# bitmagier/q-learning

Measured on AMD Instinct MI355X. Metric: env-steps/sec + grad-updates/sec, Breakout 84×84×4, 1/2/4/8 MI355X, higher is better.
Workload: dtype fp32; 1 GPU; C3: 8192 Breakout envs per GPU, replay 1000000 per GPU in HBM (prefilled), Nature-DQN (3 conv + 2 dense) in fp32, B=1024, update every 128 env-steps per GPU (replay ratio 8 samples/env-step), epsilon-greedy acting; envs_per_gpu=8192, batch=1024, replay_capacity=1000000, update_after_actions=128, parallelism=single, rccl_world=1, global_batch_per_update=1024, env_dtype=fp32 physics, u8 frames, qnet_dtype=fp32 (exact-fp32 MFMA v_mfma_f32_16x16x4_f32)

## Files before the change

### q-learning_amd/csrc/qnet32.hip

```cpp
#include <hip/hip_ext.h>
#include <hip/hip_runtime.h>

#include <algorithm>
#include <cmath>
#include <cstdlib>
#include <map>
#include <tuple>
#include <vector>

#include "objects.h"
#include "profiler.h"
#include "qnet.h"
#include "qnet32_kernels.h"
#include "update32_dev.h"

namespace qlx {

using namespace q32;

struct F32Net {
  bool bg_rows = true;
  int c1_skip = 1;
  bool update_scheduled = false;
  bool dense_partials = false;
  float partials_scale = 1.0f;
  float *fa1 = nullptr, *fa2 = nullptr, *fa3 = nullptr, *fa4 = nullptr;
  float* fpart = nullptr;
  int *frl2 = nullptr, *frl3 = nullptr;
  unsigned long long* frcnt = nullptr;
  float* fbgc = nullptr;
  uint32_t* fsteps = nullptr;
  uint8_t* fneed = nullptr;
  int fneed_ld = 0;
  uint32_t* frows2 = nullptr;
  uint8_t* fbg2 = nullptr;
  uint32_t* frows3 = nullptr;
  uint8_t* fbg3 = nullptr;
  int fparity = 0;
  int frl_cap = 0;
  int fchunk = 0;
  DeviceBuffer<uint8_t> fgrad;
  int fgrad_batch = 0;
  float *fdz1 = nullptr, *fdz2 = nullptr, *fdz3 = nullptr, *fdz4 = nullptr;
  float *fslab1 = nullptr, *fslab2 = nullptr, *fslab3 = nullptr;
  float* fpb1 = nullptr;
  float* fpbg2 = nullptr;
  float* fs2 = nullptr;
  float* fpbg3 = nullptr;
  float* fs3 = nullptr;
};

constexpr int kHeadPitch = 514;
template <int MODE, int HS = 16>
__global__ __launch_bounds__(256) void k_head32(Fc2Args A) {
  __shared__ f32x4 part[4][16];
  __shared__ float gsh[16];
  __shared__ int ash[16];
  __shared__ __attribute__((aligned(16))) float xs[16 * kHeadPitch];
  __shared__ __attribute__((aligned(16))) float w4s[512 * 3];
  typedef float f32x2 __attribute__((ext_vector_type(2)));
  const int lane = threadIdx.x & 63, wave = threadIdx.x >> 6;
  const int s0 = blockIdx.x * HS;
  const int j = lane & 15, g = lane >> 4, n = lane & 15;
  const int b = s0 + j;
  const bool valid = j < HS && b < A.B;
  const bool tail = wave == 0 && g == 0 && valid;
  const int bt = tail ? b : 0;
  int t_act = 0;
  float t_y = 0.0f, t_w = 1.0f, t_r = 0.0f, t_qs[3] = {0.0f, 0.0f, 0.0f};
  bool t_done = false;
  if (tail) {
    if (MODE == 3) {
      t_act = A.actions[bt];
      t_y = A.y[bt];
      if (A.weights) t_w = A.weights[bt];
    } else if (MODE == 2) {
      t_r = A.rewards[bt];
      t_done = A.dones[bt] != 0;
      if (A.q_select)
        for (int r = 0; r < 3; ++r) t_qs[r] = A.q_select[bt * 3 + r];
    }
// ... 418 lines not shown
  if ((int)blockIdx.x < nconv) conv_adam_block(A, N, blockIdx.x);
  else AdamDense{A, ndense}.run((int)blockIdx.x - nconv, nrm);
}

static int conv_adam_blocks() {
  int n = 0;
  for (int v = 0; v < 6; ++v) n += (kVarSize[v] + kConvAdamChunk - 1) / kConvAdamChunk;
  return n;
}



static int segs_of(int v) { return (kVarSize[v] + kNormSeg - 1) / kNormSeg; }
static_assert((1605632 + kNormSeg - 1) / kNormSeg <= kNormSegMax, "norm partials per variable");
static_assert((36864 + kNormSeg - 1) / kNormSeg <= 4 * kConvSegsPerGroup && (32768 + kNormSeg - 1) / kNormSeg <= 4 * kConvSegsPerGroup,
              "conv variable segments per conv_adam_block");
static_assert((512 * 3 + kNormSeg - 1) / kNormSeg <= 64 && (32768 + kNormSeg - 1) / kNormSeg <= 64 &&
              (36864 + kNormSeg - 1) / kNormSeg <= 64 && (8192 + kNormSeg - 1) / kNormSeg <= 64, "<= 64 partials but W3");

static int num_cus();

constexpr int kC1MaxIt = 64;
static int c1_blocks(int n) { return std::max(std::min(n, 2 * num_cus()), (n + kC1MaxIt - 1) / kC1MaxIt); }
static bool c1_one(int n) { return n <= 2048; }
static int c1_grid(int n) { return c1_one(n) ? n : c1_blocks(n); }

void f32_create(qlx_model* m) {
  F32Net& w = *(m->fp32 = new F32Net);
  const char* bg = std::getenv("QLX_F32_BG");
  w.bg_rows = !(bg && bg[0] == '0');
  const char* sk = std::getenv("QLX_F32_C1_SKIP");
  w.c1_skip = (sk && sk[0] == '0') ? 0 : 1;
}

void f32_destroy(qlx_model* m) {
  delete m->fp32;
  m->fp32 = nullptr;
}

void f32_workspace(qlx_model* m, int B) {
  F32Net& w = *m->fp32;
  const int C = std::min(B, kF32FwdChunk);
  static_assert((uint64_t)kF32FwdChunk * 12800 * 4 < 0x80000000ull, "a forward chunk's a1 stays below 2^31 bytes");
  int nseg = 0;
  for (int v = 0; v < kNumVars; ++v) nseg += segs_of(v);
  const int frl_cap = C + kListSlots * (C / std::max(1, std::min(C, 2 * num_cus())) + 1) +
                      std::max(2 * num_cus(), C / kC1MaxIt + 1) + kListSlots;
  const int need_ld = (C + 63) / 64 * 64;
  ws_alloc(m, B, [&](Arena& a) {
    w.fa1 = a.take<float>((size_t)C * 12800); w.fa2 = a.take<float>((size_t)C * 5184); w.fa3 = a.take<float>((size_t)C * 3136);
    w.fa4 = a.take<float>((size_t)B * 512);
    w.fpart = a.take<float>(nseg);
    w.frl2 = a.take<int>((size_t)frl_cap * 81); w.frl3 = a.take<int>((size_t)frl_cap * 49);
    w.frcnt = a.take<unsigned long long>(2 * 2 * kListSlots * kCntStride);
    w.fbgc = a.take<float>(160);
    w.fsteps = a.take<uint32_t>((size_t)C * 4);
    w.fneed = a.take<uint8_t>((size_t)100 * need_ld);
    w.frows2 = a.take<uint32_t>((size_t)C * 4); w.fbg2 = a.take<uint8_t>((size_t)81 * need_ld);
    w.frows3 = a.take<uint32_t>((size_t)C * 4); w.fbg3 = a.take<uint8_t>((size_t)49 * need_ld);
  });
  QLX_HIP(hipMemset(w.frcnt, 0, 2 * 2 * kListSlots * kCntStride * 8));
  w.fneed_ld = need_ld;
  w.frl_cap = frl_cap;
  w.fparity = 0;
  w.fchunk = C;
}

static void f32_grad_workspace(qlx_model* m, int B) {
  F32Net& w = *m->fp32;
  if (B <= w.fgrad_batch) return;
  QLX_HIP(hipStreamSynchronize(m->stream));
  w.fgrad.release();
  w.fgrad_batch = 0;
  auto layout = [&](Arena& a) {
    w.fdz1 = a.take<float>((size_t)B * 12800); w.fdz2 = a.take<float>((size_t)B * 5184); w.fdz3 = a.take<float>((size_t)B * 3136);
    w.fdz4 = a.take<float>((size_t)B * 512);
    w.fslab1 = a.take<float>((size_t)((B + kSC1 - 1) / kSC1) * 257 * 32);
    w.fslab2 = a.take<float>((size_t)((B + kSC2 - 1) / kSC2) * 513 * 64);
    w.fslab3 = a.take<float>((size_t)((B + kSC3 - 1) / kSC3) * 577 * 64);
    w.fpb1 = a.take<float>((size_t)((B + 15) / 16) * 400 * 32);
    w.fpbg2 = a.take<float>((size_t)((B + 15) / 16) * 81 * 64); w.fs2 = a.take<float>((size_t)((B + 15) / 16) * 64);
    w.fpbg3 = a.take<float>((size_t)((B + 15) / 16) * 49 * 64); w.fs3 = a.take<float>((size_t)((B + 15) / 16) * 64);
  };
  Arena size;
  layout(size);
  w.fgrad.alloc(size.off);
  Arena a{(uintptr_t)w.fgrad.get()};
  layout(a);
  w.fgrad_batch = B;
}

template <class P>
static void launch(qlx_model* m, const P& p, const char* scope, double work, hipStream_t s) {
  hipEvent_t ea = nullptr, eb = nullptr;
  if (m->prof) m->prof->ext(scope, work, &ea, &eb);
  hipExtLaunchKernelGGL(k_gemm32<P>, dim3(p.g.blocks()), dim3(threads_of<P>()), gemm_lds_bytes<P>(), s, ea, eb, 0u, p);
  QLX_HIP(hipGetLastError());
  debug_sync(s, scope);
}

template <class P1, class P2, class S, class T = NoSide>
static void launch_pair(qlx_model* m, const P1& p1, const P2& p2, const S& side, const char* scope, double work, hipStream_t s,
                        const T& tail = T{}) {
  const size_t lds = std::max({gemm_lds_bytes<P1>(), gemm_lds_bytes<P2>(), S::LDS, T::LDS});
  hipEvent_t ea = nullptr, eb = nullptr;
  if (m->prof) m->prof->ext(scope, work, &ea, &eb);
// ... 18 lines not shown
  return n;
}

static Grid grid(int M, int BM, int N, int BN, int nz) { return Grid{(M + BM - 1) / BM, (N + BN - 1) / BN, nz}; }

static int c1_skip(const qlx_model* m) { return m->fp32->c1_skip; }

static int balanced_whole_tiles(int M) {
  const int ncu = num_cus(), t = M / 64, whole = t - t % ncu;
  if (whole < ncu || M - whole * 64 > 32 * ncu) return 0;
  return whole;
}

template <class P, class S>
static void launch_list(qlx_model* m, const P& p, const S& side, const char* scope, double work, hipStream_t s) {
  hipEvent_t ea = nullptr, eb = nullptr;
  if (m->prof) m->prof->ext(scope, work, &ea, &eb);
  const size_t lds = std::max(gemm_lds_bytes<P>(), S::LDS);
  hipExtLaunchKernelGGL((k_gemm32_side<P, S>), dim3(side.blocks() + p.g.blocks()), dim3(threads_of<P>()), lds, s, ea, eb, 0u, p, side);
  QLX_HIP(hipGetLastError());
  debug_sync(s, scope);
}

static bool bg_rows(const qlx_model* m) { return m->fp32->bg_rows; }

static bool c1_sparse_dz(const qlx_model* m) { return bg_rows(m) && c1_skip(m); }
template <class PW, class PR, class PF>
static void conv_fwd(qlx_model* m, int M, const float* in, const float* wt, const float* bias, float* out, const char* scope,
                     double work, hipStream_t s, const PF& plain) {
  const int whole = balanced_whole_tiles(M);
  if (!whole) {
    launch(m, plain, scope, work, s);
    return;
  }
  const PW pw{Grid{whole, 1, 1}, in, wt, bias, out, M};
  const PR pr{{Grid{(M - whole * 64 + 15) / 16, 1, 1}, in, wt, bias, out, M}, whole * 4};
  launch_pair(m, pw, pr, NoSide{}, scope, work, s);
}

void f32_forward(qlx_model* m, const uint8_t* const* table, int B, hipStream_t s) {
  F32Net& w = *m->fp32;
  QLX_CHECK(m->ws_batch >= B, QLX_E_STATE, "f32 forward: workspace too small");
  m->last_batch = B;
  const float* p = m->d_params;
  for (int c0 = 0; c0 < B; c0 += w.fchunk) {
    const int n = std::min(w.fchunk, B - c0);
    const bool big = n > 2048;
    const bool lists = bg_rows(m);
    unsigned long long* cnt = w.frcnt + 2 * kListSlots * kCntStride * w.fparity;
    const bool one = c1_one(n);
    const int G = c1_grid(n);
    const int per_slot = ((G + kListSlots - 1) / kListSlots) * ((n + G - 1) / G);
    const int cap2 = per_slot * 81, cap3 = per_slot * 49;
    QLX_CHECK((size_t)kListSlots * cap2 <= w.frl_cap * 81, QLX_E_STATE, "row lists too small");
    const C1Lists L{lists ? w.frl2 : nullptr, w.frl3, cap2, cap3, cnt, w.frcnt + 2 * kListSlots * kCntStride * (w.fparity ^ 1),
                    w.fbgc, w.fsteps, w.fneed, w.fneed_ld, w.frows2, w.fbg2, w.frows3, w.fbg3};
    if (lists) w.fparity ^= 1;
    {
      const char* sc = big ? "f32_conv1_fwd_big" : "f32_conv1_fwd";
      hipEvent_t ea = nullptr, eb = nullptr;
      if (m->prof) m->prof->ext(sc, 2.0 * n * 400 * 32 * 256, &ea, &eb);
      auto kern = one ? k_conv1_fwd32<0, true> : k_conv1_fwd32<1>;
      QLX_CHECK((n + G - 1) / G <= (one ? 1 : kC1MaxIt), QLX_E_STATE, "conv1 forward: too many samples per block");
      const size_t frames = (one ? 1 : 2) * kC1Frames;
      const size_t lds = frames + 3 * kC1RmDw * 4 + (size_t)((n + G - 1) / G) * 6 * 8 + 8;
      set_lds_limit((const void*)kern, frames + 3 * kC1RmDw * 4 + (size_t)(one ? 1 : kC1MaxIt) * 6 * 8 + 8);
      hipExtLaunchKernelGGL(kern, dim3(G), dim3(256), lds, s, ea, eb, 0u, table + (size_t)c0 * 4, n,
                            p + var_offset(0), p + var_offset(1), w.fa1, c1_skip(m), L);
      QLX_HIP(hipGetLastError());
      debug_sync(s, sc);
    }
    if (lists) {
      const int nw = std::min(256, std::max(16, n / 16));
      float* c2 = w.fbgc + 32;
      float* c3 = w.fbgc + 96;
      const BgRows2 s23{{nw, w.frl2, cnt, cap2, c2, w.fa2}, {nw, w.frl3, cnt + kCntStride, cap3, c3, w.fa3}};
      auto lgrid = [&](int cap, int BM, int BN) { return Grid{1 + kListSlots * ((cap + BM - 1) / BM), 64 / BN, 1}; };
      auto run = [&](auto t2, auto t3, const char* sc2, const char* sc3) {
        using P2 = decltype(t2);
        using P3 = decltype(t3);
        const ConstRows cr{{w.fbgc, p + var_offset(2), p + var_offset(3), c2}, {c2, p + var_offset(4), p + var_offset(5), c3}};
        P2 p2{lgrid(cap2, P2::BM, P2::BN), w.fa1, p + var_offset(2), p + var_offset(3), w.fa2, w.frl2, cap2, cnt, w.fbgc};
        p2.pre_batched = big;
        launch_list(m, p2, cr, sc2, 2.0 * n * 81 * 64 * 512, s);
        launch_list(m, P3{lgrid(cap3, P3::BM, P3::BN), w.fa2, p + var_offset(4), p + var_offset(5), w.fa3, w.frl3, cap3, cnt + kCntStride, c2},
                    s23, sc3, 2.0 * n * 49 * 64 * 576, s);
      };
      if (big) {
        run(PConv2FwdL<64, 64, 2, 2>{}, PConv3FwdL<64, 64, 2, 2>{}, "f32_conv2_fwd_big", "f32_conv3_fwd_big");
        launch(m, PFc1FwdB{grid(n, PFc1FwdB::BM, 512, PFc1FwdB::BN, 1), w.fa3, p + var_offset(6), p + var_offset(7), w.fa4 + (size_t)c0 * 512, n}, "f32_fc1_fwd_big",
               2.0 * n * 3136 * 512, s);
      } else {
        run(PConv2FwdL<64, 64, 2, 2>{}, PConv3FwdL<32, 64, 2, 2>{}, "f32_conv2_fwd", "f32_conv3_fwd");
        launch(m, PFc1FwdS{grid(n, PFc1FwdS::BM, 512, PFc1FwdS::BN, 1), w.fa3, p + var_offset(6), p + var_offset(7), w.fa4 + (size_t)c0 * 512, n}, "f32_fc1_fwd",
               2.0 * n * 3136 * 512, s);
      }
    } else if (big) {
      launch(m, PConv2Fwd{grid(n * 81, 64, 64, 64, 1), w.fa1, p + var_offset(2), p + var_offset(3), w.fa2, n * 81}, "f32_conv2_fwd_big",
             2.0 * n * 81 * 64 * 512, s);
      launch(m, PConv3Fwd{grid(n * 49, 64, 64, 64, 1), w.fa2, p + var_offset(4), p + var_offset(5), w.fa3, n * 49}, "f32_conv3_fwd_big",
             2.0 * n * 49 * 64 * 576, s);
      launch(m, PFc1FwdB{grid(n, PFc1FwdB::BM, 512, PFc1FwdB::BN, 1), w.fa3, p + var_offset(6), p + var_offset(7), w.fa4 + (size_t)c0 * 512, n}, "f32_fc1_fwd_big",
             2.0 * n * 3136 * 512, s);
    } else {
      conv_fwd<PConv2Fwd, PConv2FwdR>(m, n * 81, w.fa1, p + var_offset(2), p + var_offset(3), w.fa2, "f32_conv2_fwd", 2.0 * n * 81 * 64 * 512, s,
                                      PConv2FwdS{grid(n * 81, 64, 64, 32, 1), w.fa1, p + var_offset(2), p + var_offset(3), w.fa2, n * 81});
      conv_fwd<PConv3Fwd, PConv3FwdR>(m, n * 49, w.fa2, p + var_offset(4), p + var_offset(5), w.fa3, "f32_conv3_fwd", 2.0 * n * 49 * 64 * 576, s,
                                      PConv3FwdS{grid(n * 49, 64, 64, 32, 1), w.fa2, p + var_offset(4), p + var_offset(5), w.fa3, n * 49});
      launch(m, PFc1FwdS{grid(n, PFc1FwdS::BM, 512, PFc1FwdS::BN, 1), w.fa3, p + var_offset(6), p + var_offset(7), w.fa4 + (size_t)c0 * 512, n}, "f32_fc1_fwd",
             2.0 * n * 3136 * 512, s);
    }
  }
}

void f32_head(int mode, const Fc2Args& a, int B, hipStream_t s) {
  constexpr int kHs3 = 4;
  const dim3 g((B + 15) / 16), blk(256);
  switch (mode) {
    case 0: hipLaunchKernelGGL(k_head32<0>, g, blk, 0, s, a); break;
    case 1: hipLaunchKernelGGL(k_head32<1>, g, blk, 0, s, a); break;
    case 2: hipLaunchKernelGGL(k_head32<2>, g, blk, 0, s, a); break;
    default: hipLaunchKernelGGL((k_head32<3, kHs3>), dim3((B + kHs3 - 1) / kHs3), blk, 0, s, a); break;
  }
  QLX_HIP(hipGetLastError());
  debug_sync(s, "k_head32");
}

Fc2Args f32_fc2_args(qlx_model* m, int B) {
  Fc2Args a = fc2_common(m, B);
  a.a4f = m->fp32->fa4;
  return a;
}

template <class Side>
static void f32_fc1_bwd(qlx_model* m, int B, const Side& S, hipStream_t s) {
  F32Net& w = *m->fp32;
  float* G = m->d_grads;
  const float* p = m->d_params;
  PFc1WgradS Pw{grid(3136, PFc1WgradS::BM, 512, PFc1WgradS::BN, 1), w.fa3, w.fdz4, G + var_offset(6), G + var_offset(7), B};
  PFc1DgradS Pd{grid(B, PFc1DgradS::BM, 3136, PFc1DgradS::BN, 1), w.fdz4, p + var_offset(6), w.fa3, w.fdz3, B};
  if (bg_rows(m)) {
    Pd.pbg = w.fpbg3;
    Pd.bg = w.fbg3;
    Pd.bg_ld = w.fneed_ld;
  }
  launch_pair(m, Pw, Pd, S, "f32_fc1_bwd", 2.0 * 2.0 * B * 512 * 3136, s);
// ... 281 lines not shown
```

### q-learning_amd/csrc/qnet32_kernels.h

```cpp
#pragma once
#include <hip/hip_runtime.h>

#include <cstdint>
#include <type_traits>

#include "qlx_internal.h"

namespace qlx {
namespace q32 {

typedef float f32x4 __attribute__((ext_vector_type(4)));

constexpr int BK = 32;
constexpr int kListSlots = 8;
constexpr int kCntStride = 16;

__host__ __device__ constexpr int kmaj_pad(int rows, int r) { return rows + ((r - rows % 64) % 64 + 64) % 64; }
__host__ __device__ constexpr int kmaj_pitch(int rows) {
  return kmaj_pad(rows, 48) < kmaj_pad(rows, 16) ? kmaj_pad(rows, 48) : kmaj_pad(rows, 16);
}
static_assert(kmaj_pitch(32) == 48 && kmaj_pitch(64) == 80 && kmaj_pitch(128) == 144, "KMAJ pitches");

template <int ROWS, bool KMAJ>
struct Opnd {
// ... 582 lines not shown
  static constexpr int BM = BM_, BN = BN_, WM = WM_, WN = WN_;
  static constexpr int MINW = 3;
  static constexpr bool LOAD_FENCE = !(H == 20 && BN_ == 64);
  static constexpr bool A_KMAJ = false, B_KMAJ = true, BIAS = false;
  Grid g;
  const float* in;
  const float* w;
  const float* bias;
  float* out;
  int M;
  __host__ __device__ void decode(int lb, int& tm, int& tn, int& z) const { g.decode(lb, tm, tn, z); }
  __host__ __device__ int nslabs(int) const { return KS * KS * C / BK; }
  using Streams = ConvFwdStreams<W, C, KS, OC, BM_, BN_, WM_ * WN_ * 64>;
  __device__ Streams streams(int, int row0, int col0, int tid) const {
    Streams st;
    const int m = M;
    st.a.init(in, (uint32_t)(M / (OH * OW)) * (uint32_t)(H * W * C * 4), tid, [row0, m](int r, int k) {
      const int row = row0 + r, b = row / (OH * OW), p = row - b * (OH * OW), oh = p / OW, ow = p - oh * OW;
      return row < m ? (uint32_t)(((b * H + oh * S) * W + ow * S) * C + k) * 4u : kOob;
    });
    st.init_b(w, col0, tid);
    return st;
  }
  __device__ void epi(int, int row, int col, f32x4 v) const {
#pragma unroll
    for (int r = 0; r < 4; ++r)
      if (row + r < M) out[(size_t)(row + r) * OC + col] = relu(v[r] + bias[col]);
  }
  __device__ f32x4 epi_pre(int, int, int col) const {
    const float b = bias[col];
    return f32x4{b, b, b, b};
  }
  __device__ void epi_post(int, int row, int col, f32x4 v, f32x4 b) const {
#pragma unroll
    for (int r = 0; r < 4; ++r)
      if (row + r < M) out[(size_t)(row + r) * OC + col] = relu(v[r] + b[r]);
  }
};
using PConv2Fwd = PConvFwd<20, 20, 32, 4, 2, 9, 9, 64>;
using PConv3Fwd = PConvFwd<9, 9, 64, 3, 1, 7, 7, 64>;
using PConv2FwdS = PConvFwd<20, 20, 32, 4, 2, 9, 9, 64, 64, 32, 2, 2>;
using PConv3FwdS = PConvFwd<9, 9, 64, 3, 1, 7, 7, 64, 64, 32, 2, 2>;
template <class Base>
struct RowShift : Base {
  int tm0;
  __host__ __device__ void decode(int lb, int& tm, int& tn, int& z) const {
    Base::decode(lb, tm, tn, z);
    tm += tm0;
  }
};
using PConv2FwdR = RowShift<PConvFwd<20, 20, 32, 4, 2, 9, 9, 64, 16, 64, 1, 4>>;
using PConv3FwdR = RowShift<PConvFwd<9, 9, 64, 3, 1, 7, 7, 64, 16, 64, 1, 4>>;

template <int H, int W, int C, int KS, int S, int OH, int OW, int OC, int BM_ = 64, int BN_ = 64, int WM_ = 2, int WN_ = 2,
          bool SEL = false>
struct PConvFwdL {
  static constexpr int BM = BM_, BN = BN_, WM = WM_, WN = WN_;
  static constexpr bool A_KMAJ = false, B_KMAJ = true, BIAS = false, RAW_ORDER = true;
  static constexpr bool LOAD_FENCE = true;
  static constexpr int R = OH * OW;
  using OA = Opnd<BM, false>;
  static constexpr int T = WM * WN * 64, NA = (OA::F4 + T - 1) / T;
  Grid g;
  const float* in;
  const float* w;
  const float* bias;
  float* out;
  const int* list;
  int cap;
  const unsigned long long* cnt;
  const float* cx;
  bool pre_batched = true;
  struct Pre { float b; int o[4]; };

  __host__ __device__ void decode(int lb, int& tm, int& tn, int& z) const { g.decode(lb, tm, tn, z); }
  __host__ __device__ int nslabs(int) const { return KS * KS * C / BK; }
  __device__ int count(int x) const { return (int)(cnt[x * 2 * kCntStride] >> 32); }
  template <int N>
  __device__ void entries(const int (&row)[N], int (&out)[N]) const {
    const int tm = q32_uniform(row[0] / BM);
    const int x = (tm - 1) % kListSlots, base = ((tm - 1) / kListSlots) * BM;
    const int n = count(x);
    int v[N];
#pragma unroll
    for (int i = 0; i < N; ++i) v[i] = list[x * cap + min(base + row[i] % BM, cap - 1)];
#pragma unroll
    for (int i = 0; i < N; ++i) out[i] = base + row[i] % BM < n ? v[i] : -1;
  }
  __device__ bool active(int, int row0) const {
    const int tm = row0 / BM;
    return tm != 0 && ((tm - 1) / kListSlots) * BM < count((tm - 1) % kListSlots);
  }
  __device__ Pre epi_pre(int, int row, int col) const {
    Pre q;
    q.b = bias[col];
    if (!pre_batched) {
#pragma unroll
    for (int r = 0; r < 4; ++r) {
      const int tm = (row + r) / BM;
      const int x = (tm - 1) % kListSlots, lr = ((tm - 1) / kListSlots) * BM + (row + r) % BM;
      q.o[r] = lr < count(x) ? list[x * cap + lr] : -1;
    }
    } else {
    const int rows[4] = {row, row + 1, row + 2, row + 3};
    entries(rows, q.o);
    }
    return q;
  }
  __device__ void epi_post(int, int, int col, f32x4 v, const Pre& q) const {
#pragma unroll
    for (int r = 0; r < 4; ++r)
      if (q.o[r] >= 0) out[(size_t)(q.o[r] & 0xFFFFF) * OC + col] = relu(v[r] + q.b);
  }
  using Streams = ConvFwdStreams<W, C, KS, OC, BM_, BN_, T, SEL>;
  __device__ Streams streams(int, int row0, int col0, int tid) const {
    Streams st;
    st.a.tid = tid;
    const char* lo = (const char*)in;
    const char* base = SEL && (const char*)cx < lo ? (const char*)cx : lo;
    const uint32_t in_off = (uint32_t)(lo - base), cx_off = SEL ? (uint32_t)((const char*)cx - base) : 0u;
    st.a.rs = buf_rsrc(base, kNoEnd);
    int rows[NA], raws[NA];
#pragma unroll
    for (int i = 0; i < NA; ++i) {
      int r = 0, k = 0;
      OA::coord(tid + i * T, r, k);
      rows[i] = row0 + r;
    }
    entries(rows, raws);
#pragma unroll
    for (int i = 0; i < NA; ++i) {
      int r = 0, k = 0;
      OA::coord(tid + i * T, r, k);
      const int raw = raws[i], e = raw >= 0 ? raw & 0xFFFFF : -1;
      const int bb = e / R, pp = e - bb * R, oh = pp / OW, ow = pp - oh * OW;
      st.a.vo[i] = e >= 0 ? in_off + (uint32_t)(((bb * H + oh * S) * W + ow * S) * C + k) * 4u : kOob;
      st.cxo[i] = cx_off + (uint32_t)k * 4u;
      st.msk[i] = SEL && raw >= 0 ? (uint32_t)raw >> 20 : 0u;
    }
    st.init_b(w, col0, tid);
    return st;
  }
};
template <int BM, int BN, int WM, int WN>
using PConv2FwdL = PConvFwdL<20, 20, 32, 4, 2, 9, 9, 64, BM, BN, WM, WN, false>;
template <int BM, int BN, int WM, int WN>
using PConv3FwdL = PConvFwdL<9, 9, 64, 3, 1, 7, 7, 64, BM, BN, WM, WN, true>;

template <int C, int KS, int OC>
struct PConstRow {
  static constexpr int BM = 16, BN = OC, WM = 1, WN = 4, T = 256;
  static constexpr bool A_KMAJ = false, B_KMAJ = true, BIAS = false;
  static constexpr Grid g{1, 1, 1};
  const float* cx;
  const float* w;
  const float* bias;
  float* cbuf;
  __host__ __device__ void decode(int, int& tm, int& tn, int& z) const { tm = tn = z = 0; }
  __host__ __device__ int nslabs(int) const { return KS * KS * C / BK; }
  __device__ float epi_pre(int, int, int col) const { return bias[col]; }
  __device__ void epi_post(int, int row, int col, f32x4 v, float b) const {
    if (row == 0) cbuf[col] = relu(v[0] + b);
  }
  struct Streams {
    AffineStream<BM, false, T> a;
    AffineStream<BN, true, T> b;
    struct Regs {
      typename AffineStream<BM, false, T>::Regs a;
      typename AffineStream<BN, true, T>::Regs b;
    };
    __device__ void load(int s, Regs& x) const {
      a.load((uint32_t)((s * BK) % C) * 4u, 0, x.a);
      b.load((uint32_t)s * BK * OC * 4u, 0, x.b);
    }
    __device__ void store(float* as, float* bs, const Regs& x) const {
      a.store(as, x.a);
      b.store(bs, x.b);
    }
  };
  __device__ Streams streams(int, int, int, int tid) const {
    Streams st;
    st.a.init(cx, (uint32_t)C * 4u, tid, [](int r, int k) { return r == 0 ? (uint32_t)k * 4u : kOob; });
    st.b.init(w, (uint32_t)KS * KS * C * OC * 4u, tid, [](int r, int k) { return (uint32_t)(k * OC + r) * 4u; });
    return st;
  }
};

struct ConstRows {
  using PA = PConstRow<32, 4, 64>;
  using PB = PConstRow<64, 3, 64>;
  static constexpr size_t LDS = gemm_lds_bytes<PA>();
  PA pa;
  PB pb;
  __host__ __device__ int blocks() const { return 1; }
  __device__ void run(int, float* lds) const {
    gemm_body(pa, 0, lds);
    __syncthreads();
    __threadfence();
// ... 591 lines not shown
        const int S = (min(HB, B - b0) + 3) / 4;
#pragma unroll 8
        for (int s = 0; s < S; ++s) {
          const int bl = 4 * s + g;
          const float av = t < 32 ? as[bl * 16 + n] : (n == 0 ? 1.0f : 0.0f);
          const float bv = n < 4 ? ds[bl * 4 + n] : 0.0f;
          acc = __builtin_amdgcn_mfma_f32_16x16x4f32(av, bv, acc, 0, 0, 0);
        }
      }
    }
    if (tid >= 64) return;
    if (t < 32) {
      if (n < 3)
#pragma unroll
        for (int i = 0; i < 4; ++i) dw4[(t * 16 + 4 * g + i) * 3 + n] = acc[i];
    } else if (g == 0) {
      if (n < 3) db4[n] = acc[0];
      else if (n == 3) *loss = acc[0] / (float)B;
    }
  }
};
using SideFc2 = SideFc2T<false>;
using SideFc2Dq = SideFc2T<true>;

#if !defined(QLX_Q32_POLICIES_ONLY) && !defined(QLX_Q32_NO_KERNELS)
constexpr int kC1SlotDw = 1776;
constexpr int kC1Frames = 4 * kC1SlotDw * 4;
constexpr int kC1Chunks = 4 * kFramePix / 16;

typedef const __attribute__((address_space(1))) uint8_t gbyte;
typedef unsigned int u32x4v __attribute__((ext_vector_type(4)));
typedef const __attribute__((address_space(1))) u32x4v gu4;
__device__ __forceinline__ uint4 ldg_frame(const uint8_t* f, int pos) {
  gbyte* p = f ? (gbyte*)f + pos * 16 : (gbyte*)q32_zero4;
  const u32x4v v = *(gu4*)p;
  return uint4{v.x, v.y, v.z, v.w};
}

typedef const __attribute__((address_space(4))) unsigned long long cu64;
typedef const __attribute__((address_space(4))) uint32_t cu32;
struct C1Ptrs {
  const uint8_t* p[4];
};
__device__ __forceinline__ C1Ptrs c1_ptrs(const uint8_t* const* table, int b) {
  cu64* t = (cu64*)(table + (size_t)b * 4);
  return C1Ptrs{{(const uint8_t*)t[0], (const uint8_t*)t[1], (const uint8_t*)t[2], (const uint8_t*)t[3]}};
}
__device__ __forceinline__ const uint8_t* c1_slot(const C1Ptrs& f, int slot) {
  const uint8_t* lo = (slot & 1) ? f.p[1] : f.p[0];
  const uint8_t* hi = (slot & 1) ? f.p[3] : f.p[2];
  return (slot & 2) ? hi : lo;
}

__device__ __forceinline__ void c1_prefetch(const C1Ptrs& f, uint4 (&pf)[7]) {
#pragma unroll
  for (int j = 0; j < 7; ++j) {
    const int q = threadIdx.x + 256 * j;
    const bool ok = q < kC1Chunks;
    const int qq = ok ? q : 0, slot = qq / 441, pos = qq - slot * 441;
    pf[j] = ldg_frame(ok ? c1_slot(f, slot) : nullptr, pos);
  }
}
__device__ __forceinline__ void c1_put(uint32_t* dst, int q, const uint4& v) {
  const int slot = q / 441, pos = q - slot * 441, bx = pos / 21, by = pos - bx * 21;
  uint32_t* d = dst + slot * kC1SlotDw + 4 * bx * 21 + by;
  d[0] = v.x;
  d[21] = v.y;
  d[42] = v.z;
  d[63] = v.w;
}
__device__ __forceinline__ void c1_stage(uint32_t* dst, const uint4 (&pf)[7]) {
#pragma unroll
  for (int j = 0; j < 7; ++j) {
    const int q = threadIdx.x + 256 * j;
    if (q < kC1Chunks) c1_put(dst, q, pf[j]);
  }
}
__device__ __forceinline__ float ubyte(uint32_t w, int i) { return (float)((w >> (8 * i)) & 0xFFu); }

struct C1Lists {
  int* rl2;
  int* rl3;
  int cap2, cap3;
  unsigned long long* cnt;
  unsigned long long* cnt_next;
  float* xbg;
  uint32_t* steps;
  uint8_t* need;
  int need_ld;
  uint32_t* rows2;
  uint8_t* bg2;
  uint32_t* rows3;
  uint8_t* bg3;
};
constexpr int kC1RmDw = 24;

__device__ __forceinline__ int c1_opaque_tid() {
  int t = threadIdx.x;
  asm volatile("" : "+v"(t));
  return t;
}
__device__ __forceinline__ void c1_mark(uint32_t* rm, const uint4 (&pf)[7]) {
  const int t = c1_opaque_tid();
#pragma unroll
  for (int j = 0; j < 7; ++j) {
    const int q = t + 256 * j;
    if (q < kC1Chunks && (pf[j].x | pf[j].y | pf[j].z | pf[j].w) != 0u) {
      const int pos = q % 441, bx = pos / 21, by = pos - bx * 21;
      atomicOr(&rm[bx], 1u << by);
    }
  }
}

__device__ __forceinline__ void c1_steps(const uint32_t* rm, uint32_t* out, uint8_t* need, int need_ld, int b, int lane) {
  bool nd[2];
#pragma unroll
  for (int h = 0; h < 2; ++h) {
    const int s = lane + 64 * h;
    const bool valid = s < 100;
    const int ss = valid ? s : 0, oh = ss / 5, t = ss - 5 * oh;
    nd[h] = valid && ((((rm[oh] | rm[oh + 1]) >> (4 * t)) & 0x1Fu) != 0u);
    if (need && valid) need[(size_t)s * need_ld + b] = nd[h] ? 1 : 0;
  }
  const unsigned long long m0 = __builtin_amdgcn_ballot_w64(nd[0]), m1 = __builtin_amdgcn_ballot_w64(nd[1]);
  if (lane < 4) {
    const unsigned long long m = lane < 2 ? m0 : m1;
    out[lane] = (uint32_t)(m >> (32 * (lane & 1)));
  }
}
__device__ __forceinline__ bool c1_step_set(unsigned long long lo, unsigned long long hi, int st) {
  return ((st < 64 ? lo >> st : hi >> (st - 64)) & 1ull) != 0ull;
}
__device__ __forceinline__ uint32_t c1_tiles(const uint32_t* rm, int lane) {
  const int t = lane < 25 ? lane : 0, bx = 4 * (t / 5), by = 4 * (t % 5);
  uint32_t mm = 0;
#pragma unroll
  for (int r = 0; r < 5; ++r) mm |= rm[bx + r];
  return (uint32_t)__builtin_amdgcn_ballot_w64(lane < 25 && ((mm >> by) & 0x1Fu) != 0u);
}
__device__ __forceinline__ void c1_flags(const uint32_t* rm, unsigned long long* cl, int wave, const C1Lists& L, int b) {
  const int tid = c1_opaque_tid();
  const int R = wave < 2 ? 81 : 49, p = wave < 2 ? tid : tid - 128;
  const bool valid = p < R;
  const int pp = valid ? p : 0;
  bool nonbg;
  if (wave < 2) {
    const int i = pp / 9, j = pp - 9 * i;
    uint32_t mm = 0;
#pragma unroll
    for (int r = 0; r < 5; ++r) mm |= rm[2 * i + r];
    nonbg = ((mm >> (2 * j)) & 0x1Fu) != 0u;
  } else {
    const int i = pp / 7, j = pp - 7 * i;
    uint32_t mm = 0;
#pragma unroll
    for (int r = 0; r < 9; ++r) mm |= rm[2 * i + r];
    nonbg = ((mm >> (2 * j)) & 0x1FFu) != 0u;
  }
  const unsigned long long bn = __builtin_amdgcn_ballot_w64(valid && nonbg), bb = __builtin_amdgcn_ballot_w64(valid && !nonbg);
  if ((tid & 63) == 0) {
    cl[0] = bn;
    cl[1] = bb;
  }
  if (wave < 2 && L.rows2) {
    const int lane = tid & 63;
    if (lane < 2 && (wave == 0 || lane == 0)) L.rows2[(size_t)b * 4 + 2 * wave + lane] = (uint32_t)(bn >> (32 * lane));
    if (wave == 1 && lane == 1) L.rows2[(size_t)b * 4 + 3] = 0u;
    if (valid) L.bg2[(size_t)p * L.need_ld + b] = nonbg ? 0 : 1;
  }
  if (wave == 2 && L.rows3) {
    const int lane = tid & 63;
    if (lane < 4) L.rows3[(size_t)b * 4 + lane] = lane < 2 ? (uint32_t)(bn >> (32 * lane)) : 0u;
    if (valid) L.bg3[(size_t)p * L.need_ld + b] = nonbg ? 0 : 1;
  }
}
__device__ __forceinline__ void c1_lists_flush(const unsigned long long* cl, int nit, int b0, int G, const C1Lists& L, int wave,
                                               int tid, unsigned long long* xch) {
  const int lane = tid & 63, R = wave < 2 ? 81 : 49, p = wave < 2 ? tid : tid - 128;
  int* rl = wave < 2 ? L.rl2 : L.rl3;
  auto wave_tot = [&](int wv) {
    unsigned long long t = 0;
    for (int it = 0; it < nit; ++it)
      t += ((unsigned long long)__builtin_popcountll(cl[(it * 3 + wv) * 2]) << 32) |
           (unsigned long long)__builtin_popcountll(cl[(it * 3 + wv) * 2 + 1]);
    return t;
  };
  unsigned long long old = 0;
  const int slot = blockIdx.x % kListSlots, cap = wave < 2 ? L.cap2 : L.cap3;
  rl += slot * cap;
  if ((wave == 0 || wave == 2) && lane == 0) {
    const unsigned long long tot = wave == 0 ? wave_tot(0) + wave_tot(1) : wave_tot(2);
    old = __hip_atomic_fetch_add(L.cnt + (slot * 2 + (wave < 2 ? 0 : 1)) * kCntStride, tot, __ATOMIC_RELAXED, __HIP_MEMORY_SCOPE_AGENT);
    if (wave == 0) *xch = old;
  }
  __syncthreads();
  if (wave == 1) old = *xch + wave_tot(0);
  if (wave >= 3) return;
  old = __shfl(old, 0);
  int on = (int)(old >> 32), og = (int)(uint32_t)old;
  const unsigned long long below = (1ull << lane) - 1ull;
  for (int it = 0; it < nit; ++it) {
    const unsigned long long bn = cl[(it * 3 + wave) * 2], bb = cl[(it * 3 + wave) * 2 + 1];
    const int e = (b0 + it * G) * R + p;
    int tap = 0;
    if (wave == 2) {
      const unsigned long long g0 = cl[(it * 3) * 2 + 1], g1 = cl[(it * 3 + 1) * 2 + 1];
      const int i = p / 7, j = p - 7 * (p / 7);
#pragma unroll
      for (int t = 0; t < 9; ++t) {
        const int q = (i + t / 3) * 9 + j + t % 3;
        tap |= (int)(((q < 64 ? g0 >> q : g1 >> (q - 64)) & 1ull) << t);
      }
    }
    if ((bn >> lane) & 1ull) rl[on + __builtin_popcountll(bn & below)] = e | (tap << 20);
    else if ((bb >> lane) & 1ull) rl[cap - 1 - (og + __builtin_popcountll(bb & below))] = e;
    on += __builtin_popcountll(bn);
    og += __builtin_popcountll(bb);
  }
}

__device__ __forceinline__ void c1_fwd_sample(const uint32_t* fr, uint32_t lb, int nt, int rp, int g, int col,
                                              const float (&wf)[64], float bias, int skip, uint32_t live, float* a1, int b) {
  {
    const unsigned long long every = skip == 0 ? ~0ull : 0ull;
    auto tile_live = [&](int j) { return ((live >> (rp + 2 * j)) & 1u) != 0u; };
    auto tile_dwords = [&](int j, uint32_t (&d)[16]) {
      const int t = rp + 2 * j;
      const uint32_t base = lb + (uint32_t)((t / 5) * (16 * 21) + (t % 5) * 4);
#pragma unroll
      for (int kq = 0; kq < 16; ++kq) d[kq] = fr[base + (kq >> 1) * 21 + (kq & 1)];
    };
    const uint32_t so = (uint32_t)(g * 20 * 32 + col);
    const float zb = relu(0.0f + bias);
    auto tile = [&](int j, const uint32_t (&d)[16], uint32_t (&dn)[16]) {
      const bool lv = tile_live(j), nx = j + 1 < nt && tile_live(j + 1);
      const int t = rp + 2 * j;
      float* at = a1 + ((size_t)b * 400 + 80 * (t / 5) + 4 * (t % 5)) * 32;
      if (lv) {
        bool nz[16];
#pragma unroll
        for (int kq = 0; kq < 16; ++kq) nz[kq] = (__builtin_amdgcn_ballot_w64(d[kq] != 0u) | every) != 0ull;
        if (nx) tile_dwords(j + 1, dn);
        f32x4 acc = zero4();
#pragma unroll
        for (int kq = 0; kq < 16; ++kq)
          if (nz[kq])
#pragma unroll
            for (int kw = 0; kw < 4; ++kw) acc = __builtin_amdgcn_mfma_f32_16x16x4f32(ubyte(d[kq], kw), wf[kq * 4 + kw], acc, 0, 0, 0);
#pragma unroll
        for (int i = 0; i < 4; ++i) at[so + 32u * i] = relu(acc[i] + bias);
      } else {
        if (nx) tile_dwords(j + 1, dn);
#pragma unroll
        for (int i = 0; i < 4; ++i) at[so + 32u * i] = zb;
      }
    };
    uint32_t dd[14][16];
    if (tile_live(0)) tile_dwords(0, dd[0]);
#pragma unroll
    for (int j = 0; j < 13; ++j)
      if (j < nt) tile(j, dd[j], dd[j + 1]);
  }
}

constexpr int kC1OneMinW = 4;
template <int ROLE, bool ONE = false>
__global__ __launch_bounds__(256, ONE ? kC1OneMinW : 2) void k_conv1_fwd32(const uint8_t* const* table, int B, const float* w0,
                                                                           const float* b0, float* a1, int skip, const C1Lists L) {
  extern __shared__ __attribute__((aligned(16))) uint32_t c1w[];
  uint32_t* rm = c1w + (ONE ? 1 : 2) * 4 * kC1SlotDw;
  unsigned long long* cl = reinterpret_cast<unsigned long long*>(rm + 3 * kC1RmDw);
  const bool lists = L.rl2 != nullptr;
  const bool marks = lists || L.rows2 != nullptr || L.rows3 != nullptr;
  const int tid = threadIdx.x, lane = tid & 63;
  const int wave = __builtin_amdgcn_readfirstlane(tid >> 6);
  if (marks) {
    if (blockIdx.x == 0 && tid < 2 * kListSlots) L.cnt_next[tid * kCntStride] = 0ull;
    if (blockIdx.x == 0 && tid < 32) L.xbg[tid] = relu(0.0f + b0[tid]);
    if (tid < 3 * kC1RmDw) rm[tid] = 0u;
    __syncthreads();
  }
  const int ct = wave & 1, rp = wave >> 1;
  const int col = ct * 16 + (lane & 15), g = lane >> 4;
  float wf[64];
#pragma unroll
  for (int kk = 0; kk < 64; ++kk) wf[kk] = w0[(kk * 4 + g) * 32 + col];
  const float bias = b0[col];
  const uint32_t lb = (uint32_t)(g * kC1SlotDw + 4 * ((lane & 15) >> 2) * 21 + (lane & 3));
  const int nt = rp == 0 ? 13 : 12;
  int b = blockIdx.x;
  if (b >= B) return;
  if constexpr (ONE) {
    {
      uint4 pf[7];
      c1_prefetch(c1_ptrs(table, b), pf);
      c1_stage(c1w, pf);
      if (marks) c1_mark(rm, pf);
    }
    __syncthreads();
    c1_fwd_sample(c1w, lb, nt, rp, g, col, wf, bias, skip, marks && skip != 0 ? c1_tiles(rm, lane) : ~0u, a1, b);
    if (marks) {
      if (wave < 3) c1_flags(rm, cl + wave * 2, wave, L, b);
      else if (L.steps) c1_steps(rm, L.steps + (size_t)b * 4, L.need, L.need_ld, b, lane);
      if (lists) {
        __syncthreads();
        c1_lists_flush(cl, 1, blockIdx.x, gridDim.x, L, wave, tid, cl + 6);
      }
    }
    return;
  }
  uint4 pf[7];
  c1_prefetch(c1_ptrs(table, b), pf);
  C1Ptrs nxt = c1_ptrs(table, b + (int)gridDim.x < B ? b + (int)gridDim.x : b);
  c1_stage(c1w, pf);
  if (marks) c1_mark(rm, pf);
  __syncthreads();
  for (int it = 0; b < B; b += gridDim.x, ++it) {
    const uint32_t* fr = c1w + (it & 1) * (4 * kC1SlotDw);
    const int nb = b + gridDim.x;
    if (nb < B) {
      c1_prefetch(nxt, pf);
      nxt = c1_ptrs(table, nb + (int)gridDim.x < B ? nb + (int)gridDim.x : nb);
    }
    if (marks && wave == 3 && tid - 192 < kC1RmDw) rm[((it + 2) % 3) * kC1RmDw + tid - 192] = 0u;
    c1_fwd_sample(fr, lb, nt, rp, g, col, wf, bias, skip, marks && skip != 0 ? c1_tiles(rm + (it % 3) * kC1RmDw, lane) : ~0u, a1,
                  b);
    if (marks && wave < 3) c1_flags(rm + (it % 3) * kC1RmDw, cl + it * 6 + wave * 2, wave, L, b);
    if (marks && wave == 3 && L.steps) c1_steps(rm + (it % 3) * kC1RmDw, L.steps + (size_t)b * 4, L.need, L.need_ld, b, lane);
    if (nb < B) {
      c1_stage(c1w + ((it + 1) & 1) * (4 * kC1SlotDw), pf);
      if (marks) c1_mark(rm + ((it + 1) % 3) * kC1RmDw, pf);
    }
    __syncthreads();
  }
  if (lists) {
    const int nit = (B - (int)blockIdx.x + (int)gridDim.x - 1) / (int)gridDim.x;
    c1_lists_flush(cl, nit, blockIdx.x, gridDim.x, L, wave, tid, cl + nit * 6);
  }
}

constexpr int kC1DzChunks = 400 * 32 / 4;
constexpr int kC1WgSlotDw = 1768;
constexpr int kC1WgradThreads = 512;
constexpr int kC1WgradPf = (kC1Chunks + kC1DzChunks + kC1WgradThreads - 1) / kC1WgradThreads;
constexpr size_t kC1WgradLds = (size_t)4 * kC1WgSlotDw * 4 + (size_t)400 * 32 * 4;
__host__ __device__ constexpr int c1_wgrad_blocks(int nz) { return nz; }
__global__ __launch_bounds__(kC1WgradThreads, 2) void k_conv1_wgrad32(const uint8_t* const* table, const float* dz1, int B, int nz,
                                                                       float* slab, int skip, const uint32_t* steps,
                                                                       const float* pb) {
  extern __shared__ __attribute__((aligned(16))) uint32_t c1w[];
  float* dzs = reinterpret_cast<float*>(c1w + 4 * kC1WgSlotDw);
  const int tid = threadIdx.x, lane = tid & 63;
  const int wave = __builtin_amdgcn_readfirstlane(tid >> 6);
  const int z = blockIdx.x, hh = wave >> 2, wq = wave & 3;
  const int g = lane >> 4, l15 = lane & 15;
  const int b0 = z * QLX_F32_WGRAD_CHUNK_CONV1;
  const int nb = min(QLX_F32_WGRAD_CHUNK_CONV1, B - b0);
  const int ao = (l15 & 3) * kC1WgSlotDw + (2 * wq + (l15 >> 3)) * 21 + ((l15 >> 2) & 1);
  const int bo = hh * 16 + l15;
  const int pxo = ao + g, dzo = hh * 6400 + g * 16 + l15;
  const unsigned long long every = skip == 0 ? ~0ull : 0ull;

  const int boc = tid & 31, bjb = tid >> 5;
  float bt = 0.0f;
  {
    const int NR = ((B + 15) >> 4) * 400, R = (NR + nz - 1) / nz, i0 = z * R, i1 = min(NR, i0 + R);
    for (int i = i0 + bjb; i < i1; i += 64) {
      float v[4];
#pragma unroll
      for (int u = 0; u < 4; ++u) v[u] = i + 16 * u < i1 ? pb[(size_t)(i + 16 * u) * 32 + boc] : 0.0f;
#pragma unroll
      for (int u = 0; u < 4; ++u)
        if (i + 16 * u < i1) bt = __fadd_rn(bt, v[u]);
    }
// ... 109 lines not shown
```

Measured before the change: 332,900 env-steps/s.

## Precompute conv row-list window offsets in conv1 and simplify frame prefetch addressing

```diff
diff --git a/q-learning_amd/csrc/qnet32.hip b/q-learning_amd/csrc/qnet32.hip
--- a/q-learning_amd/csrc/qnet32.hip
+++ b/q-learning_amd/csrc/qnet32.hip
@@ -27,6 +27,7 @@
   float *fa1 = nullptr, *fa2 = nullptr, *fa3 = nullptr, *fa4 = nullptr;
   float* fpart = nullptr;
   int *frl2 = nullptr, *frl3 = nullptr;
+  uint32_t *frw2 = nullptr, *frw3 = nullptr;
   unsigned long long* frcnt = nullptr;
   float* fbgc = nullptr;
   uint32_t* fsteps = nullptr;
@@ -551,6 +552,7 @@
     w.fa4 = a.take<float>((size_t)B * 512);
     w.fpart = a.take<float>(nseg);
     w.frl2 = a.take<int>((size_t)frl_cap * 81); w.frl3 = a.take<int>((size_t)frl_cap * 49);
+    w.frw2 = a.take<uint32_t>((size_t)frl_cap * 81); w.frw3 = a.take<uint32_t>((size_t)frl_cap * 49);
     w.frcnt = a.take<unsigned long long>(2 * 2 * kListSlots * kCntStride);
     w.fbgc = a.take<float>(160);
     w.fsteps = a.take<uint32_t>((size_t)C * 4);
@@ -675,9 +677,10 @@
     const int G = c1_grid(n);
     const int per_slot = ((G + kListSlots - 1) / kListSlots) * ((n + G - 1) / G);
     const int cap2 = per_slot * 81, cap3 = per_slot * 49;
-    QLX_CHECK((size_t)kListSlots * cap2 <= w.frl_cap * 81, QLX_E_STATE, "row lists too small");
+    QLX_CHECK((size_t)kListSlots * cap2 <= (size_t)w.frl_cap * 81 && (size_t)kListSlots * cap3 <= (size_t)w.frl_cap * 49, QLX_E_STATE,
+              "row lists too small");
     const C1Lists L{lists ? w.frl2 : nullptr, w.frl3, cap2, cap3, cnt, w.frcnt + 2 * kListSlots * kCntStride * (w.fparity ^ 1),
-                    w.fbgc, w.fsteps, w.fneed, w.fneed_ld, w.frows2, w.fbg2, w.frows3, w.fbg3};
+                    w.fbgc, w.fsteps, w.fneed, w.fneed_ld, w.frows2, w.fbg2, w.frows3, w.fbg3, w.frw2, w.frw3};
     if (lists) w.fparity ^= 1;
     {
       const char* sc = big ? "f32_conv1_fwd_big" : "f32_conv1_fwd";
@@ -703,10 +706,9 @@
         using P2 = decltype(t2);
         using P3 = decltype(t3);
         const ConstRows cr{{w.fbgc, p + var_offset(2), p + var_offset(3), c2}, {c2, p + var_offset(4), p + var_offset(5), c3}};
-        P2 p2{lgrid(cap2, P2::BM, P2::BN), w.fa1, p + var_offset(2), p + var_offset(3), w.fa2, w.frl2, cap2, cnt, w.fbgc};
-        p2.pre_batched = big;
+        const P2 p2{lgrid(cap2, P2::BM, P2::BN), w.fa1, p + var_offset(2), p + var_offset(3), w.fa2, w.frl2, cap2, cnt, w.fbgc, w.frw2};
         launch_list(m, p2, cr, sc2, 2.0 * n * 81 * 64 * 512, s);
-        launch_list(m, P3{lgrid(cap3, P3::BM, P3::BN), w.fa2, p + var_offset(4), p + var_offset(5), w.fa3, w.frl3, cap3, cnt + kCntStride, c2},
+        launch_list(m, P3{lgrid(cap3, P3::BM, P3::BN), w.fa2, p + var_offset(4), p + var_offset(5), w.fa3, w.frl3, cap3, cnt + kCntStride, c2, w.frw3},
                     s23, sc3, 2.0 * n * 49 * 64 * 576, s);
       };
       if (big) {
@@ -714,7 +716,7 @@
         launch(m, PFc1FwdB{grid(n, PFc1FwdB::BM, 512, PFc1FwdB::BN, 1), w.fa3, p + var_offset(6), p + var_offset(7), w.fa4 + (size_t)c0 * 512, n}, "f32_fc1_fwd_big",
                2.0 * n * 3136 * 512, s);
       } else {
-        run(PConv2FwdL<64, 64, 2, 2>{}, PConv3FwdL<32, 64, 2, 2>{}, "f32_conv2_fwd", "f32_conv3_fwd");
+        run(PConv2FwdL<64, 64, 2, 2, false>{}, PConv3FwdL<32, 64, 2, 2>{}, "f32_conv2_fwd", "f32_conv3_fwd");
         launch(m, PFc1FwdS{grid(n, PFc1FwdS::BM, 512, PFc1FwdS::BN, 1), w.fa3, p + var_offset(6), p + var_offset(7), w.fa4 + (size_t)c0 * 512, n}, "f32_fc1_fwd",
                2.0 * n * 3136 * 512, s);
       }
diff --git a/q-learning_amd/csrc/qnet32_kernels.h b/q-learning_amd/csrc/qnet32_kernels.h
--- a/q-learning_amd/csrc/qnet32_kernels.h
+++ b/q-learning_amd/csrc/qnet32_kernels.h
@@ -658,8 +658,17 @@
 using PConv2FwdR = RowShift<PConvFwd<20, 20, 32, 4, 2, 9, 9, 64, 16, 64, 1, 4>>;
 using PConv3FwdR = RowShift<PConvFwd<9, 9, 64, 3, 1, 7, 7, 64, 16, 64, 1, 4>>;
 
+
+template <int H, int W, int C, int S, int OW>
+__host__ __device__ inline uint32_t list_window(int b, int p) {
+  const int oh = p / OW, ow = p - oh * OW;
+  return (uint32_t)(((b * H + oh * S) * W + ow * S) * C) * 4u;
+}
+__host__ __device__ inline uint32_t list_window2(int b, int p) { return list_window<20, 20, 32, 2, 9>(b, p); }
+__host__ __device__ inline uint32_t list_window3(int b, int p) { return list_window<9, 9, 64, 1, 7>(b, p); }
+
 template <int H, int W, int C, int KS, int S, int OH, int OW, int OC, int BM_ = 64, int BN_ = 64, int WM_ = 2, int WN_ = 2,
-          bool SEL = false>
+          bool SEL = false, bool PRE_BATCHED = true>
 struct PConvFwdL {
   static constexpr int BM = BM_, BN = BN_, WM = WM_, WN = WN_;
   static constexpr bool A_KMAJ = false, B_KMAJ = true, BIAS = false, RAW_ORDER = true;
@@ -676,10 +685,14 @@
   int cap;
   const unsigned long long* cnt;
   const float* cx;
-  bool pre_batched = true;
+  const uint32_t* win;
   struct Pre { float b; int o[4]; };
 
-  __host__ __device__ void decode(int lb, int& tm, int& tn, int& z) const { g.decode(lb, tm, tn, z); }
+  __host__ __device__ void decode(int lb, int& tm, int& tn, int& z) const {
+    tn = lb % (OC / BN);
+    tm = lb / (OC / BN);
+    z = 0;
+  }
   __host__ __device__ int nslabs(int) const { return KS * KS * C / BK; }
   __device__ int count(int x) const { return (int)(cnt[x * 2 * kCntStride] >> 32); }
   template <int N>
@@ -700,7 +713,7 @@
   __device__ Pre epi_pre(int, int row, int col) const {
     Pre q;
     q.b = bias[col];
-    if (!pre_batched) {
+    if constexpr (!PRE_BATCHED) {
 #pragma unroll
     for (int r = 0; r < 4; ++r) {
       const int tm = (row + r) / BM;
@@ -726,30 +739,34 @@
     const char* base = SEL && (const char*)cx < lo ? (const char*)cx : lo;
     const uint32_t in_off = (uint32_t)(lo - base), cx_off = SEL ? (uint32_t)((const char*)cx - base) : 0u;
     st.a.rs = buf_rsrc(base, kNoEnd);
-    int rows[NA], raws[NA];
+    const int tm = q32_uniform(row0 / BM);
+    const int x = (tm - 1) % kListSlots, lr0 = ((tm - 1) / kListSlots) * BM;
+    const int n = count(x) - lr0, last = cap - 1 - lr0;
+    const uint32_t* wl = win + x * cap + lr0;
+    const int* el = list + x * cap + lr0;
+    uint32_t wv[NA];
+    int raws[NA];
 #pragma unroll
     for (int i = 0; i < NA; ++i) {
       int r = 0, k = 0;
       OA::coord(tid + i * T, r, k);
-      rows[i] = row0 + r;
-    }
-    entries(rows, raws);
+      wv[i] = wl[min(r, last)];
+      if (SEL) raws[i] = el[min(r, last)];
+    }
 #pragma unroll
     for (int i = 0; i < NA; ++i) {
       int r = 0, k = 0;
       OA::coord(tid + i * T, r, k);
-      const int raw = raws[i], e = raw >= 0 ? raw & 0xFFFFF : -1;
-      const int bb = e / R, pp = e - bb * R, oh = pp / OW, ow = pp - oh * OW;
-      st.a.vo[i] = e >= 0 ? in_off + (uint32_t)(((bb * H + oh * S) * W + ow * S) * C + k) * 4u : kOob;
+      st.a.vo[i] = r < n ? in_off + wv[i] + (uint32_t)k * 4u : kOob;
       st.cxo[i] = cx_off + (uint32_t)k * 4u;
-      st.msk[i] = SEL && raw >= 0 ? (uint32_t)raw >> 20 : 0u;
+      st.msk[i] = SEL && r < n ? (uint32_t)raws[i] >> 20 : 0u;
     }
     st.init_b(w, col0, tid);
     return st;
   }
 };
-template <int BM, int BN, int WM, int WN>
-using PConv2FwdL = PConvFwdL<20, 20, 32, 4, 2, 9, 9, 64, BM, BN, WM, WN, false>;
+template <int BM, int BN, int WM, int WN, bool PRE_BATCHED = true>
+using PConv2FwdL = PConvFwdL<20, 20, 32, 4, 2, 9, 9, 64, BM, BN, WM, WN, false, PRE_BATCHED>;
 template <int BM, int BN, int WM, int WN>
 using PConv3FwdL = PConvFwdL<9, 9, 64, 3, 1, 7, 7, 64, BM, BN, WM, WN, true>;
 
@@ -1447,13 +1464,36 @@
   return (slot & 2) ? hi : lo;
 }
 
+constexpr bool c1_two_frames(int T, int n) {
+  for (int j = 0; j < n; ++j)
+    if ((T * j + T - 1) / 441 > (T * j) / 441 + 1) return false;
+  return true;
+}
+static_assert(c1_two_frames(256, 7), "a load instruction's chunks: at most two frames");
+__device__ __forceinline__ gbyte* c1_chunk_addr(const C1Ptrs& f, int q0, int T, int q) {
+  const int slo = q0 / 441, shi = (q0 + T - 1) / 441;
+  auto live = [&](int s) { return s < 4 && f.p[s & 3] != nullptr; };
+  auto base = [&](int s) { return live(s) ? (gbyte*)f.p[s & 3] : (gbyte*)q32_zero4; };
+  auto mask = [&](int s) { return live(s) ? ~0u : 0u; };
+  if (slo == shi) return base(slo) + ((uint32_t)((q - 441 * slo) * 16) & mask(slo));
+  const bool hi = q >= 441 * shi;
+  gbyte* b = hi ? base(shi) : base(slo);
+  return b + ((uint32_t)((q - (hi ? 441 * shi : 441 * slo)) * 16) & (hi ? mask(shi) : mask(slo)));
+}
+
+template <bool TWO>
 __device__ __forceinline__ void c1_prefetch(const C1Ptrs& f, uint4 (&pf)[7]) {
 #pragma unroll
   for (int j = 0; j < 7; ++j) {
     const int q = threadIdx.x + 256 * j;
-    const bool ok = q < kC1Chunks;
-    const int qq = ok ? q : 0, slot = qq / 441, pos = qq - slot * 441;
-    pf[j] = ldg_frame(ok ? c1_slot(f, slot) : nullptr, pos);
+    if constexpr (TWO) {
+      const u32x4v v = *(gu4*)c1_chunk_addr(f, 256 * j, 256, q);
+      pf[j] = uint4{v.x, v.y, v.z, v.w};
+    } else {
+      const bool ok = q < kC1Chunks;
+      const int qq = ok ? q : 0, slot = qq / 441, pos = qq - slot * 441;
+      pf[j] = ldg_frame(ok ? c1_slot(f, slot) : nullptr, pos);
+    }
   }
 }
 __device__ __forceinline__ void c1_put(uint32_t* dst, int q, const uint4& v) {
@@ -1487,6 +1527,8 @@
   uint8_t* bg2;
   uint32_t* rows3;
   uint8_t* bg3;
+  uint32_t* rw2;
+  uint32_t* rw3;
 };
 constexpr int kC1RmDw = 24;
 
@@ -1583,6 +1625,9 @@
   unsigned long long old = 0;
   const int slot = blockIdx.x % kListSlots, cap = wave < 2 ? L.cap2 : L.cap3;
   rl += slot * cap;
+  uint32_t* rw = (wave < 2 ? L.rw2 : L.rw3) + slot * cap;
+  const int q3 = wave == 2 && p < 49 ? (p / 7) * 9 + p % 7 : 0;
+  const uint32_t pw = wave < 2 ? list_window2(0, p) : list_window3(0, p), bw = wave < 2 ? list_window2(1, 0) : list_window3(1, 0);
   if ((wave == 0 || wave == 2) && lane == 0) {
     const unsigned long long tot = wave == 0 ? wave_tot(0) + wave_tot(1) : wave_tot(2);
     old = __hip_atomic_fetch_add(L.cnt + (slot * 2 + (wave < 2 ? 0 : 1)) * kCntStride, tot, __ATOMIC_RELAXED, __HIP_MEMORY_SCOPE_AGENT);
@@ -1600,15 +1645,14 @@
     int tap = 0;
     if (wave == 2) {
       const unsigned long long g0 = cl[(it * 3) * 2 + 1], g1 = cl[(it * 3 + 1) * 2 + 1];
-      const int i = p / 7, j = p - 7 * (p / 7);
-#pragma unroll
-      for (int t = 0; t < 9; ++t) {
-        const int q = (i + t / 3) * 9 + j + t % 3;
-        tap |= (int)(((q < 64 ? g0 >> q : g1 >> (q - 64)) & 1ull) << t);
-      }
-    }
-    if ((bn >> lane) & 1ull) rl[on + __builtin_popcountll(bn & below)] = e | (tap << 20);
-    else if ((bb >> lane) & 1ull) rl[cap - 1 - (og + __builtin_popcountll(bb & below))] = e;
+      const unsigned long long v = (g0 >> q3) | ((g1 << 1) << (63 - q3));
+      tap = (int)((v & 7ull) | (((v >> 9) & 7ull) << 3) | (((v >> 18) & 7ull) << 6));
+    }
+    if ((bn >> lane) & 1ull) {
+      const int at = on + __builtin_popcountll(bn & below);
+      rl[at] = e | (tap << 20);
+      rw[at] = pw + (uint32_t)(b0 + it * G) * bw;
+    } else if ((bb >> lane) & 1ull) rl[cap - 1 - (og + __builtin_popcountll(bb & below))] = e;
     on += __builtin_popcountll(bn);
     og += __builtin_popcountll(bb);
   }
@@ -1688,7 +1732,7 @@
   if constexpr (ONE) {
     {
       uint4 pf[7];
-      c1_prefetch(c1_ptrs(table, b), pf);
+      c1_prefetch<false>(c1_ptrs(table, b), pf);
       c1_stage(c1w, pf);
       if (marks) c1_mark(rm, pf);
     }
@@ -1705,7 +1749,7 @@
     return;
   }
   uint4 pf[7];
-  c1_prefetch(c1_ptrs(table, b), pf);
+  c1_prefetch<true>(c1_ptrs(table, b), pf);
   C1Ptrs nxt = c1_ptrs(table, b + (int)gridDim.x < B ? b + (int)gridDim.x : b);
   c1_stage(c1w, pf);
   if (marks) c1_mark(rm, pf);
@@ -1714,7 +1758,7 @@
     const uint32_t* fr = c1w + (it & 1) * (4 * kC1SlotDw);
     const int nb = b + gridDim.x;
     if (nb < B) {
-      c1_prefetch(nxt, pf);
+      c1_prefetch<true>(nxt, pf);
       nxt = c1_ptrs(table, nb + (int)gridDim.x < B ? nb + (int)gridDim.x : nb);
     }
     if (marks && wave == 3 && tid - 192 < kC1RmDw) rm[((it + 2) % 3) * kC1RmDw + tid - 192] = 0u;
```

Result: no change. 334,800 env-steps/s, median of 6 (+0.6%).
